# seveirbian/go-libp2p-pubsub

Measured on AMD Instinct MI355X. Metric: peer-message deliveries/sec + gossipsub rounds/sec (node), 1M peers 64 topics, higher is better.
Workload: dtype f64+u64; 1 GPU; config4: 1M peers, 64 topics, k=32, gossipsub v1.1 + Eth2 scoring, 1000 msgs/round, 10 hops/round; peers=1000000, topics=64, degree=32, msgs_per_round=1000, hops_per_round=10, parallelism=replicas1

## Files before the change

### go-libp2p-pubsub_amd/csrc/gs_engine.hip

```cpp
#include "gs_engine.h"

static thread_local std::string g_err;
void gs_set_error(const std::string& msg) { g_err = msg; }

static std::vector<int32_t> partition_bounds(const std::vector<int64_t>& rowptr, int N, int world) {
  const int64_t E = rowptr[N];
  std::vector<int32_t> part(world + 1, N);
  part[0] = 0;
  for (int r = 1; r < world; ++r)
    part[r] = (int32_t)(std::lower_bound(rowptr.begin(), rowptr.begin() + N, (E * r) / world) - rowptr.begin());
  for (int r = 1; r <= world; ++r) part[r] = std::max(part[r], part[r - 1]);
  return part;
}

static TopicP to_dev(const gs_topic_score_params& p, bool scored) {
  TopicP t{};
  t.TopicWeight = p.TopicWeight;
  t.TimeInMeshWeight = p.TimeInMeshWeight;
  t.TimeInMeshQuantum = p.TimeInMeshQuantum ? p.TimeInMeshQuantum : 1;
  t.TimeInMeshCap = p.TimeInMeshCap;
  t.FmdWeight = p.FirstMessageDeliveriesWeight;
  t.FmdDecay = p.FirstMessageDeliveriesDecay;
  t.FmdCap = p.FirstMessageDeliveriesCap;
  t.MmdWeight = p.MeshMessageDeliveriesWeight;
// ... 445 lines not shown
int gs_engine::allocIwantPool() {
  Dev& x = d;
  poolSeg = cfg.router == GS_ROUTER_GOSSIPSUB ? std::max<int64_t>((1 << 24) / world, 4 * eOwn) : 16;
  poolSeg = (poolSeg + 63) & ~63ll;
  x.poolCap = (int64_t)(rank + 1) * poolSeg;
  int sub = 1;
  while (world == 1 && sub < 256 && (poolSeg / (2 * sub)) >= (1 << 20)) sub *= 2;
  x.poolSub = sub;
  x.poolSubCap = poolSeg / sub;
  x.poolBase0 = (int64_t)rank * poolSeg;
  x.poolS0Mask = -1;
  if (const char* dbg = std::getenv("GS_DEBUG_POOL_SUB_CAP"))
    if (world == 1) {
      x.poolSubCap = std::min<int64_t>(x.poolSubCap, std::max<long long>(1, std::atoll(dbg)));
      x.poolS0Mask = 0;
      std::fprintf(stderr, "gossip engine: GS_DEBUG_POOL_SUB_CAP=%s active (IWANT sub-arenas of %lld ids, "
                   "sub-arena 0 first; a test-only setting)\n", dbg, (long long)x.poolSubCap);
    }
  for (int k = 0; k < 2; ++k) x.pool[k] = dalloc<int32_t>((size_t)poolSeg * world);
  x.poolCnt = dalloc<unsigned long long>((size_t)2 * x.poolSub * 16);
  x.cutSpK = dalloc<unsigned long long>(GS_CUTSPILL); x.cutSpM = dalloc<int64_t>(GS_CUTSPILL);
  x.cutSpN = dalloc<unsigned long long>(1);
  if (doPX) {
    for (int k = 0; k < 2; ++k) x.cPx[k] = ralloc<int64_t>(0xFF);
    x.pxqCap = std::max<int64_t>(1 << 16, 4 * (int64_t)N);
    x.pxq = dalloc<unsigned long long>((size_t)x.pxqCap); x.pxqN = dalloc<unsigned long long>(1);
  }
  x.slotSrc = dalloc<int32_t>(S, 0xFF); x.slotPubHop = dalloc<int64_t>(S); x.slotMid = dalloc<int64_t>(S, 0xFF);
  x.slotKind = dalloc<uint8_t>(S);
  return GS_OK;
}

int gs_engine::allocAdversary(const Plan& pl) {
  Dev& x = d;
  if (!behaveAll) return GS_OK;
  uint8_t* b = dalloc<uint8_t>(N);
  GS_TRY(putNow(b, behaveH.data(), (size_t)N));
  x.behave = b;
  if (!(behaveAll & GS_BEHAVE_IWANT_SPAM)) return GS_OK;
  for (int k = 0; k < 2; ++k) {
    x.cSpam[k] = ralloc<int64_t>(0xFF);
    x.cNSrv[k] = ralloc<uint8_t>();
  }
  x.pmaskRow = dalloc<int32_t>(N);
  x.pmask = dalloc<uint64_t>((size_t)pl.nSpam * S);
  x.spamRow = ealloc<int32_t>();
  for (int k = 0; k < 2; ++k) x.pflag[k] = dalloc<uint8_t>((size_t)poolSeg * world);
  x.spamCnt = dalloc<uint32_t>((size_t)std::max<int64_t>(pl.nSpamEdges, 1) * (S / 8));
  GS_TRY(putNow(x.pmaskRow, pl.pmaskRowH.data(), (size_t)N));
  return putEdges(x.spamRow, spamRowH);
}

int gs_engine::allocGater(const Plan& pl) {
  Dev& x = d;
  if (!gaterOn) return GS_OK;
  x.gThreshold = gaterP.Threshold; x.gGlobalDecay = gaterP.GlobalDecay; x.gSourceDecay = gaterP.SourceDecay;
  x.gDecayToZero = gaterP.DecayToZero; x.gDupW = gaterP.DuplicateWeight; x.gIgnW = gaterP.IgnoreWeight;
  x.gRejW = gaterP.RejectWeight; x.gQuiet = gaterP.Quiet;
  x.gValidate = dalloc<double>(N); x.gThrottle = dalloc<double>(N); x.gLast = dalloc<int64_t>(N);
  x.gSt = ealloc<double>(0, 4);
  x.gGrp = ealloc<uint8_t>();
  x.gConn = ealloc<int32_t>(); x.gExp = ealloc<int64_t>();
  std::vector<uint8_t> grp(E);
  for (int u = 0; u < N; ++u)
    for (int64_t e = rowptr[u]; e < rowptr[u + 1]; ++e) {
      const uint32_t ip = ipv4.empty() ? 0u : ipv4[col[e]];
      int64_t f = rowptr[u];
      while ((ipv4.empty() ? 0u : ipv4[col[f]]) != ip) ++f;
      grp[e] = (uint8_t)(f - rowptr[u]);
    }
  std::vector<int64_t> never(N, INT64_MIN);
  std::vector<int32_t> conn((size_t)E, 0);
  for (int u = 0; u < N; ++u)
    for (int64_t e = rowptr[u]; e < rowptr[u + 1]; ++e)
      if (!pl.isDown(e)) conn[rowptr[u] + grp[e]]++;
  GS_TRY(putEdges(x.gConn, conn));
  GS_TRY(putEdges(x.gGrp, grp));
  return putNow(x.gLast, never.data(), (size_t)N);
}

int gs_engine::allocReadback() {
  Dev& x = d;
#ifdef GS_STAMPS
  x.stamps = dalloc<unsigned long long>((size_t)(N / 1024 + 1) * 24);
#endif
  x.pad = dalloc<double>(256 * 64 * 2);
  x.ctr = dalloc<unsigned long long>((size_t)C_NCOUNTERS * GS_CTR_SPREAD); x.err = dalloc<int32_t>(1);
  dScoreTmp = ealloc<double>();
  dHopOut = dalloc<int32_t>(N); dFromOut = dalloc<int32_t>(N);
  return GS_OK;
}

int gs_engine::allocLatency() {
  if (!latOn) return GS_OK;
  const size_t bins = (size_t)latBins();
  d.latCnt = dalloc<uint32_t>((size_t)S);
  dLatM = dalloc<uint32_t>((size_t)S * bins);
  dLatH = dalloc<unsigned long long>((size_t)T * bins);
  int cus = 0;
  HIPCHECK(hipDeviceGetAttribute(&cus, hipDeviceAttributeMultiprocessorCount, cfg.device));
  const unsigned fit = (unsigned)(GS_LAT_CU_LDS / std::max<size_t>((size_t)S * 4, 1));
  latGrid = std::min<unsigned>(std::max(fit, 1u), GS_LAT_WGS_PER_CU) * (unsigned)std::max(cus, 1);
  return GS_OK;
}

int gs_engine::allocTrace() {
  Dev& x = d;
  if (traceMask.empty()) return GS_OK;
  uint8_t* tm = dalloc<uint8_t>(N);
  x.trace = dalloc<gs_trace_event>((size_t)traceCap);
  x.traceN = dalloc<unsigned long long>(1);
  x.traceCap = traceCap;
  GS_TRY(putNow(tm, traceMask.data(), (size_t)N));
  x.traced = tm;
  for (int u = n0; u < n1; ++u) {
    if (!traceMask[u]) continue;
    auto up = [&](int64_t e) { return !dormant.count({std::min(u, col[e]), std::max(u, col[e])}); };
    for (int64_t e = rowptr[u]; e < rowptr[u + 1]; ++e)
      if (up(e))
        tracePending.push_back(gs_trace_event{0, -1, GS_TRACE_ADD_PEER, u, col[e], -1, 0, mixed ? protoH[e] : (uint8_t)0});
    for (int t = 0; t < T; ++t)
      if ((sub[u] >> t) & 1) tracePending.push_back(gs_trace_event{0, -1, GS_TRACE_JOIN, u, -1, (int16_t)t, 0, 0});
    for (int64_t e = rowptr[u]; e < rowptr[u + 1]; ++e)
      if (up(e)) hostRpc(GS_TRACE_RECV_RPC, u, col[e], 0, GS_RPC_ORD(0, GS_RPC_O_HELLO), -1, sub[col[e]], 1);
  }
  return GS_OK;
}

int gs_engine::allocPartition() {
  Dev& x = d;
  if (world == 1) return GS_OK;
  x.xmark = ealloc<uint8_t>();
  uint8_t* nr = dalloc<uint8_t>(N);
  xCnt = dalloc<unsigned long long>(gsx::XCnt::words(world));
  xOff = dalloc<int64_t>(world);
  xpCnt = dalloc<unsigned long long>(gsx::XpCnt::words(world));
  xpOff = dalloc<int64_t>(gsx::XpOff::words(world));
  std::vector<uint8_t> h(N);
  for (int r = 0; r < world; ++r)
    for (int v = part[r]; v < part[r + 1]; ++v) h[v] = (uint8_t)r;
  GS_TRY(putNow(nr, h.data(), (size_t)N));
  x.nodeRank = nr;
  HIPCHECK(hipHostMalloc((void**)&xHost, gsx::Readback::words(world) * 8, hipHostMallocDefault));
  return GS_OK;
}

int gs_engine::initConnections(const Plan& pl) {
  if (!events.empty() || doPX || !dormant.empty()) GS_TRY(enableChurn());
  if (dormant.empty()) return GS_OK;
  std::vector<uint8_t> al((size_t)E, 1);
  for (int64_t e = 0; e < E; ++e)
    if (pl.downH[e]) al[e] = aliveH[e] = 0;
  GS_TRY(putNow(d.alive, al.data(), (size_t)E));
  if (d.rstate) GS_TRY(putNow(d.rstate, al.data(), (size_t)E));
  return GS_OK;
}

int gs_engine::allocAcct(const Plan& pl) {
  Dev& x = d;
  if (!acctOn) return GS_OK;
  x.rpcB = ealloc<unsigned long long>(); x.rpcN = ealloc<unsigned long long>();
  AcctT* ac = dalloc<AcctT>(T);
  GS_TRY(allocFail("RPC accounting"));
  const uint64_t bo = (uint64_t)(gp.PruneBackoff / kSec);
  std::vector<AcctT> ah(T);
  for (int t = 0; t < T; ++t) {
    ah[t].msgF = (int32_t)gs_pb_field(acctMsg[t]);
// ... 1610 lines not shown
```

### go-libp2p-pubsub_amd/csrc/gs_kernels.h

```cpp
#pragma once
#include <type_traits>

#include "gs_device.h"

#define GS_SB 8
#ifndef GS_RB
#define GS_RB 4
#endif
#define GS_RP 1024
__device__ __forceinline__ int rp_pad(int pl) { return pl + (pl >> 6); }
__host__ __device__ __forceinline__ int score_wave_edges(int T) { return T * 64 <= GS_RP ? 64 : GS_RP / T; }
#define GS_SCW 256
template <int MODE, bool LANE_T>
__global__ __launch_bounds__(64) void k_score_rows(Dev d, double* __restrict__ out) {
  __shared__ double sT[GS_RP + GS_RP / 64];
  __shared__ uint16_t sList[GS_SCW];
  const int lane = lane_id();
  const int T = d.T;
  const int sgw = score_wave_edges(T);
  const int64_t eb = d.e0 + (int64_t)blockIdx.x * GS_SCW;
  int nNeed = 0;
#pragma unroll
  for (int k = 0; k < GS_SCW / 64; ++k) {
    const int64_t e = eb + 64 * k + lane;
// ... 444 lines not shown
  const int slot = d.mSlot[b + i];
  atomicOr((unsigned long long*)&d.pubmask[cur][slot >> 6], 1ull << (slot & 63));
}

__device__ __forceinline__ void rs_select(const Dev& d, int u, int64_t base, int deg, int p, uint64_t subp, int slot,
                                          int ff) {
  const int lane = lane_id();
  const int t = slot / d.St;
  const int origin = d.slotSrc[slot];
  const bool cand = lane < deg && ((subp >> t) & 1) && lane != ff && p != origin;
  const bool fs = cand && d.proto != nullptr && d.proto[base + lane] == GS_PROTO_FLOODSUB;
  const bool rc = cand && !fs;
  const int n = __popcll(__ballot(rc));
  bool sel = cand;
  if (n > 6) {
    int target = d.rsTarget < n ? d.rsTarget : n;
    if (target < n) {
      const uint64_t key = gs_key64(d.seed, GS_SITE_RANDOMSUB, u, (uint32_t)d.slotMid[slot], p, 0);
      sel = fs || select_k(rc, key, target);
    }
  }
  const unsigned long long m = __ballot(sel);
  if (lane == 0) d.sel[(int64_t)u * d.S + slot] = m;
}
__device__ __forceinline__ void rs_select2(const Dev& d, int u, int64_t base, int deg, int pIn, uint64_t subpIn,
                                           int slotA, int ffA, int slotB, int ffB) {
  const int lane = lane_id();
  const int h = lane >> 5, el = lane & 31;
  const int p = __shfl(pIn, el);
  const uint64_t subp = shfl_u64(subpIn, el);
  const int slot = h ? slotB : slotA;
  const int ff = h ? ffB : ffA;
  const int t = slot / d.St;
  const int origin = d.slotSrc[slot];
  const bool cand = el < deg && ((subp >> t) & 1) && el != ff && p != origin;
  const bool fs = cand && d.proto != nullptr && d.proto[base + el] == GS_PROTO_FLOODSUB;
  const bool rc = cand && !fs;
  const int n = __popc((uint32_t)(__ballot(rc) >> (32 * h)));
  bool sel = cand;
  const int target = d.rsTarget < n ? d.rsTarget : n;
  if (n > 6 && target < n) {
    const uint64_t key = gs_key64(d.seed, GS_SITE_RANDOMSUB, u, (uint32_t)d.slotMid[slot], p, 0);
    sel = fs || select_k_half(rc, key, target);
  }
  const unsigned long long m = __ballot(sel);
  if (lane == 0) d.sel[(int64_t)u * d.S + slotA] = m & 0xFFFFFFFFull;
  if (lane == 32) d.sel[(int64_t)u * d.S + slotB] = m >> 32;
}

struct WMask {
  uint64_t m[4];
};
__device__ __forceinline__ bool wm_has(const WMask& a, int w) { return (a.m[w >> 6] >> (w & 63)) & 1; }
__device__ __forceinline__ int wm_rank(const WMask& a, int w) {
  int r = 0;
  for (int k = 0; k < (w >> 6); ++k) r += __popcll(a.m[k]);
  return r + __popcll(a.m[w >> 6] & ((1ull << (w & 63)) - 1));
}

__device__ __forceinline__ unsigned long long wave_sum_ll(long long v) {
  for (int o = 32; o > 0; o >>= 1) v += __shfl_xor(v, o);
  return (unsigned long long)v;
}

#define GS_NO_SLOT 0x7FFFFFFF

#ifdef GS_STAMPS
#define GS_STAMP_AT(region, k, val)                                                                \
  do {                                                                                             \
    if ((blockIdx.x & 1023) == 0 && lane == 0) {                                                   \
      const int64_t _i = ((int64_t)d.N / 1024 + 1) * 8 * (region) + (blockIdx.x >> 10) * 8 + (k);  \
      if ((k) >= 0 && (k) < 8 && _i < ((int64_t)d.N / 1024 + 1) * 24) d.stamps[_i] = (val);        \
      else set_err(d, E_STAMP);                                                                    \
    }                                                                                              \
  } while (0)
#define GS_STAMP(k) GS_STAMP_AT(0, k, clock64())
#define GS_STAMPB(k) GS_STAMP_AT(1, k, clock64())
#define GS_STAMPH(k, v) GS_STAMP_AT(2, k, v)
#define GS_STAMPB_CLEAR()                                  \
  do {                                                     \
    for (int _k = 0; _k < 8; ++_k) GS_STAMP_AT(1, _k, 0ull); \
  } while (0)
#define GS_CLK() clock64()
#else
#define GS_STAMPH(k, v) \
  do {                  \
  } while (0)
#define GS_CLK() 0ull
#define GS_STAMP(k) \
  do {              \
  } while (0)
#define GS_STAMPB(k) \
  do {               \
  } while (0)
#define GS_STAMPB_CLEAR() \
  do {                    \
  } while (0)
#endif

template <bool ADV>
using PhaseADev = std::conditional_t<ADV, const Dev*, Dev>;
__device__ __forceinline__ const Dev& dev_of(const Dev& d) { return d; }
__device__ __forceinline__ const Dev& dev_of(const Dev* d) { return *d; }
#ifndef GS_WPE_PA_WIDE
#define GS_WPE_PA_WIDE 4
#endif
template <bool NARROW, bool ADV>
constexpr int pa_waves = (!NARROW && !ADV) ? GS_WPE_PA_WIDE : GS_WPE_PA;
template <int WPL, bool NARROW, bool ADV, bool DENSE = false>
__global__ __launch_bounds__(64) __attribute__((amdgpu_waves_per_eu(pa_waves<NARROW, ADV>))) void k_phase_a(
    PhaseADev<ADV> dArg, int64_t h, int cur, int head,
                                                WMask amR, WMask amW, WMask amP, WMask amF, int nR, int nY) {
  static_assert(!(DENSE && ADV), "the dense pass 1 is honest-only");
  const Dev& d = dev_of(dArg);
  extern __shared__ __attribute__((aligned(16))) uint32_t smem32[];
  const int nCnt = (d.T * d.maxDeg + 7) & ~7;
  const int nCntW = NARROW ? nCnt / 2 : nCnt;
  uint32_t* scnt = smem32;
  uint64_t* sD = (uint64_t*)(scnt + nCntW);
  const int cT = d.T;
  auto cword = [&](int i, int t) -> int { return NARROW ? (i * cT + t) >> 1 : i * cT + t; };
  uint64_t* sYm = sD + nR;
  uint16_t* sRk = (uint16_t*)(sYm + nR);
  uint16_t* sYp = sRk + d.W;
  uint8_t* sFirst = (uint8_t*)(sYm + nR) + ((2 * (d.W + nR) + 15) & ~15);
  uint32_t* sUnc = (uint32_t*)(sFirst + nY);
  const int prow = (ADV && d.pmaskRow != nullptr) ? d.pmaskRow[d.n0 + blockIdx.x] : -1;
  const bool hasUnc = d.needAge || (ADV && d.pmaskRow != nullptr);
  uint32_t* sInv = sUnc + (hasUnc ? nCnt : 0);
  uint32_t* sPer = sInv + nCnt;
  double* sGThr = (double*)(sPer + 4 * 64);
  uint64_t* sDrop = (uint64_t*)(sGThr + 64);
  __shared__ uint64_t sStart[GS_BMAP];
  __shared__ uint64_t sComp[64];
  __shared__ uint64_t sRelay[64], sPub[64];
  __shared__ int sSnd[64];
  __shared__ uint32_t sAddr[64];
  __shared__ uint32_t sQ[GS_QCAP];
  const int v = d.n0 + blockIdx.x;
  const int lane = lane_id();
  const int prv = cur ^ 1;
  const int W = d.W;
  const int T = d.T;
  const int FC = d.FC;
  const int64_t base = d.rowptr[v];
  const int deg = (int)(d.rowptr[v + 1] - base);
  const uint64_t sv = d.sub[v];
  const bool valid = lane < deg;
  const bool gossipV = gossip_host(d, v);
  const bool scoring = d.scoring != 0 && gossipV;
  int u = 0, jr = -1, Ln = 0;
  int64_t pOff = -1;
  uint64_t relay = 0, pub = 0, relayAll = 0, pubAll = 0;
  bool gray = false;
  int irOff = 0, irN = 0;
  if (valid) {
    const int64_t e = base + lane;
    u = d.col[e];
    jr = d.jrIn[e];
    const ulonglong2 fw = d.fwdIn[prv][e];
    relayAll = fw.x;
    pubAll = fw.y;
    relay = relayAll & sv;
    pub = pubAll & sv;
    const int64_t ir = d.cIresp[prv][e];
    if (ir >= 0) {
      irOff = (int)(ir >> 24);
      irN = (int)(ir & 0xFFFFFF);
    }
    gray = scoring && !d.direct[e] && d.score0[e] < d.graylistThr;
    if (relayAll | pubAll) {
      if (d.ibxRec[0] != nullptr) {
        const int64_t rec = d.ibxRec[prv][e];
        if (rec >= 0) {
          pOff = rec >> 24;
          Ln = (int)(rec & 0xFFFFFF);
        }
      }
      if (pOff < 0) Ln = d.fln[prv][u];
    }
  }
  bool liveD = false, authU = false;
  int exD = 0;
  if constexpr (DENSE) {
    authU = valid && d.nAuth[u] > 0;
    if (valid && (relayAll | pubAll)) {
      liveD = d.fbN[prv][u] != 0 && (relayAll != 0 || authU);
      exD = d.fex[prv][d.rev[base + lane]];
    }
    Ln = 0;
  }
  const uint64_t authM = __ballot(authU);
  const uint64_t pushM = __ballot(pOff >= 0);
  GS_STAMP(0);
  const bool authV = d.nAuth[v] > 0;
  for (int k = lane; k < nCntW / 4; k += 64) ((uint4*)scnt)[k] = make_uint4(0, 0, 0, 0);
  const bool acct = d.rpcB != nullptr;
  if (hasUnc)
    for (int k = lane; k < nCnt / 4; k += 64) ((uint4*)sUnc)[k] = make_uint4(0, 0, 0, 0);
  for (int k = lane; k < nR; k += 64) {
    sD[k] = 0;
    sYm[k] = d.yTab[k];
    sYp[k] = (uint16_t)d.yTab[d.W + k];
  }
  {
    int rb = 0;
#pragma unroll
    for (int j = 0; j < GS_MAX_WPL; ++j) {
      const uint64_t m = amR.m[j];
      if (64 * j + lane < W)
        sRk[64 * j + lane] = ((m >> lane) & 1) ? (uint16_t)(rb + __popcll(m & ((1ull << lane) - 1))) : (uint16_t)0xFFFF;
      rb += __popcll(m);
    }
  }
  for (int k = lane; k < nY / 16; k += 64) ((uint4*)sFirst)[k] = make_uint4(~0u, ~0u, ~0u, ~0u);
  bool ctlGated = false;
  int nSrvRpc = 0;
  if constexpr (ADV) {
    for (int k = lane; k < nCnt / 4; k += 64) ((uint4*)sInv)[k] = make_uint4(0, 0, 0, 0);
    for (int k = lane; k < 4 * 64; k += 64) sPer[k] = 0;
    for (int k = lane; k < nR; k += 64) sDrop[k] = 0;
    double thr = -1.0;
    if (d.gater && gossipV && valid && !gray && !d.direct[base + lane]) {
      const int64_t last = d.gLast[v];
      const double gv = d.gValidate[v], gt = d.gThrottle[v];
      const bool active = !(last == INT64_MIN || h * d.hop_ns - last > d.gQuiet) && gt != 0 &&
                          !(gv != 0 && gt / gv < d.gThreshold);
      if (active) {
        const int64_t ge = base + d.gGrp[base + lane];
        const double de = d.gSt[ge], du = d.gSt[d.eOwn + ge], ig = d.gSt[2 * d.eOwn + ge], rj = d.gSt[3 * d.eOwn + ge];
        const double total = de + d.gDupW * du + d.gIgnW * ig + d.gRejW * rj;
        if (total != 0) thr = (1 + de) / (1 + total);
      }
    }
    sGThr[lane] = thr;
    if (valid && thr >= 0 && (d.cPre[prv][base + lane] != 0 || d.cHb[prv][base + lane] != 0)) {
      const double uu = gs_key_to_unit(gs_key64(d.seed, GS_SITE_GATER, v, u, (uint32_t)h, 0xFFFFFFFFu));
      ctlGated = !(uu < thr);
    }
    if (valid && d.cNSrv[prv] != nullptr) nSrvRpc = d.cNSrv[prv][base + lane];
    else if (irN) nSrvRpc = 1;
  }
  constexpr int EPBP = 8;
  const int nb = pOff >= 0 ? (Ln + EPBP - 1) / EPBP : (Ln + 3) >> 2;
  const int bincl = wave_incl_sum(nb);
  const int totalBlk = wave_last(bincl);
  const int nNE = __popcll(__ballot(nb > 0));
  {
    const uint64_t ne = __ballot(nb > 0);
    for (int k = lane; k < GS_BMAP; k += 64) sStart[k] = 0ull;
    __syncthreads();
    const int fb = bincl - nb;
    if (nb > 0) {
      sComp[__popcll(ne & ((1ull << lane) - 1))] =
          (uint64_t)(unsigned)fb | ((uint64_t)lane << 24) | ((uint64_t)(unsigned)Ln << 32);
      if (fb < 64 * GS_BMAP) atomicOr((unsigned long long*)&sStart[fb >> 6], 1ull << (fb & 63));
    }
  }
  sRelay[lane] = relay;
  sPub[lane] = pub;
  sSnd[lane] = valid ? (u | (jr << 24) | (rs_host(d, u) ? (1 << 30) : 0) | (gray ? (1 << 31) : 0)) : 0;
  sAddr[lane] = pOff >= 0 ? (uint32_t)(pOff >> 3) : (uint32_t)u * (uint32_t)FC;
  const uint64_t scoredT = __ballot(lane < T && scoring && d.tp[lane].scored);
  constexpr int PF3 = 16;
  const int nWdPf = (NARROW && scoring && d.dltN != nullptr) ? (deg * T) >> 1 : 0;
  const bool pf3 = nWdPf > 0 && nWdPf <= 64 * PF3;
  uint32_t q3[PF3];
  if (pf3) {
    const uint32_t* const pw = (const uint32_t*)(d.dltN + base * T);
#pragma unroll
    for (int k = 0; k < PF3; ++k) {
      const int wi = lane + 64 * k;
      q3[k] = pw[wi < nWdPf ? wi : nWdPf - 1];
    }
  }
  uint64_t Sp[WPL], Hp[WPL], Op[WPL];
#pragma unroll
  for (int j = 0; j < WPL; ++j) {
    const int w = lane + 64 * j;
    Sp[j] = Hp[j] = Op[j] = 0;
    if constexpr (!ADV) {
      const bool act = w < W && wm_has(amR, w);
      if (act || (w < W && wm_has(amP, w))) Sp[j] = d.seen[(int64_t)v * W + w];
      if (act) {
        Op[j] = d.oldm[w];
        if (gossipV) Hp[j] = d.hist[((int64_t)head * d.nOwnH + (v - d.n0)) * W + w];
      }
    }
  }
  __syncthreads();
  GS_STAMP(1);

  int nSent = 0, nGray = 0;
  long long nCopies = 0;
  int nGatedCopies = 0;
  uint64_t throttled = 0;
  auto kindOf = [&](int slot, int t) -> int {
    if constexpr (!ADV) return GS_MSG_VALID;
    return ((d.topicVal >> t) & 1) ? (int)d.slotKind[slot] : GS_MSG_VALID;
  };
  auto gated = [&](int i, int slot) -> bool {
    if constexpr (!ADV) return false;
    const double thr = sGThr[i];
    if (thr < 0) return false;
    const uint32_t mid = (uint32_t)d.slotMid[slot];
    const double uu = gs_key_to_unit(gs_key64(d.seed, GS_SITE_GATER, v, d.col[base + i], (uint32_t)h, mid));
    return !(uu < thr);
  };
  const bool trv = is_traced(d, v);
  auto deliver = [&](int i, int slot, bool payloadRpc) {
    if (payloadRpc && gated(i, slot)) {
      ++nGatedCopies;
      throttled |= 1ull << i;
      return;
    }
    const int w = slot >> 6;
    const int t = (int)__umulhi((unsigned)slot, d.stMagic);
    if (trv) trace_emit(d, h, GS_TRACE_COPY, v, d.col[base + i], t, d.slotMid[slot], 2);
    const int kind = kindOf(slot, t);
    if constexpr (ADV) {
      atomicAdd(&sPer[i], 1u);
      if (kind == GS_MSG_REJECT) atomicAdd(&sInv[i * T + t], 1u);
    }
    if (kind == GS_MSG_VALID) {
      if (NARROW) {
        const int pl = i * T + t;
        atomicAdd(&scnt[cword(i, t)], 1u << (16 * (pl & 1)));
      } else {
        atomicAdd(&scnt[cword(i, t)], 1u);
      }
    }
    ++nCopies;
    const int rk = sRk[w];
    const uint64_t ym = rk == 0xFFFF ? 0ull : sYm[rk];
    const bool young = (ym >> (slot & 63)) & 1;
    unsigned long long pold = 0;
    if (prow >= 0 && kind == GS_MSG_VALID)
      pold = atomicOr((unsigned long long*)&d.pmask[(int64_t)prow * d.S + slot], 1ull << i);
    if (d.needAge || !young || prow >= 0) {
      const bool had = (d.seen[(int64_t)v * W + w] >> (slot & 63)) & 1;
      if (had && kind == GS_MSG_VALID) {
        bool unc = (pold >> i) & 1;
        if (d.needAge && !unc) {
          const int64_t firstHop = d.slotPubHop[slot] + d.age[(int64_t)v * d.S + slot];
          unc = (h - firstHop) * d.hop_ns > d.tp[t].MmdWindow;
        }
        if (unc) atomicAdd(&sUnc[i * T + t], 1u);
      }
      if (!young) {
        if (!had) set_err(d, E_LATE);
        return;
      }
    }
    const int ix = sYp[rk] + __popcll(ym & ((1ull << (slot & 63)) - 1));
    atomicOr((unsigned long long*)&sD[rk], 1ull << (slot & 63));
    uint32_t* wp = (uint32_t*)(sFirst + (ix & ~3));
    const int sh = 8 * (ix & 3);
    uint32_t old = *wp;
    while ((int)((old >> sh) & 0xFF) > i) {
      const uint32_t nw = (old & ~(0xFFu << sh)) | ((uint32_t)i << sh);
      const uint32_t prev = atomicCAS(wp, old, nw);
      if (prev == old) break;
      old = prev;
    }
  };
  const uint32_t* const flPrv = prv ? d.fl[1] : d.fl[0];
  const uint16_t* const ibxPrv = prv ? d.ibx[1] : d.ibx[0];
  auto load_block = [&](int i, int kb) -> uint4 {
    if ((pushM >> i) & 1) return *(const uint4*)(ibxPrv + 8 * (size_t)sAddr[i] + 8 * kb);
    return *(const uint4*)(flPrv + (size_t)sAddr[i] + 4 * kb);
  };
  auto walk = [&](auto&& fn, bool count) {
    int qh = 0, qt = 0;
    int rankPrev = -1;
    constexpr int PB = 8;
    for (int b0 = 0; b0 < totalBlk; b0 += 64 * PB) {
      int si[PB], kb[PB];
      uint4 q[PB];
#pragma unroll
      for (int rr = 0; rr < PB; ++rr) {
        const int B = b0 + rr * 64;
        const int bidx = B + lane;
        si[rr] = -1;
        kb[rr] = 0;
        q[rr] = make_uint4(0, 0, 0, 0);
        if (B < 64 * GS_BMAP) {
          const uint64_t mb = sStart[B >> 6];
          const int rank = rankPrev + __popcll(mb & ((2ull << lane) - 1));
          rankPrev += __popcll(mb);
          if (bidx < totalBlk) {
            const uint64_t ce = sComp[rank];
            si[rr] = (int)((ce >> 24) & 63);
            const int k = bidx - (int)(ce & 0xFFFFFF);
            kb[rr] = k | (int)((ce >> 32) << 16);
            q[rr] = load_block(si[rr], k);
          }
        } else if (bidx < totalBlk) {
          int lo = 0, hi = nNE - 1;
          while (lo < hi) {
            const int mid = (lo + hi + 1) >> 1;
            if ((int)(sComp[mid] & 0xFFFFFF) <= bidx) lo = mid; else hi = mid - 1;
          }
          const uint64_t ce = sComp[lo];
          si[rr] = (int)((ce >> 24) & 63);
          const int k = bidx - (int)(ce & 0xFFFFFF);
          kb[rr] = k | (int)((ce >> 32) << 16);
          q[rr] = load_block(si[rr], k);
        }
      }
#pragma unroll
      for (int rr = 0; rr < PB; ++rr) {
        if (b0 + rr * 64 >= totalBlk) break;
        uint32_t en[EPBP];
        bool sn[EPBP];
        bool wide = false;
        {
          const int i = si[rr] < 0 ? 0 : si[rr];
          const int snd = sSnd[i];
          const int uu = snd & 0xFFFFFF;
          const int jri = (snd >> 24) & 0x3F;
          const bool rsS = (snd >> 30) & 1;
          const bool isGray = snd < 0;
          const uint64_t rl = sRelay[i], pb = sPub[i];
          const bool pushed = (pushM >> i) & 1;
          const int epb = pushed ? EPBP : 4;
          const int n = si[rr] < 0 ? 0 : min(epb, (kb[rr] >> 16) - epb * (kb[rr] & 0xFFFF));
          wide = n > 4;
#pragma unroll
          for (int c = 4; c < EPBP; ++c) {
            sn[c] = false;
            en[c] = 0;
          }
          if (pushed) {
#pragma unroll
            for (int c = 0; c < EPBP; ++c) {
              const uint32_t wd = c < 2 ? q[rr].x : c < 4 ? q[rr].y : c < 6 ? q[rr].z : q[rr].w;
              const int slot = (int)((c & 1) ? (wd >> 16) : (wd & 0xFFFFu));
              const int t = (int)__umulhi((unsigned)slot, d.stMagic);
              const bool sent = c < n && !(authV && d.slotSrc[slot] == v);
              if (count) {
                nSent += sent;
                if (sent && isGray) ++nGray;
              }
              sn[c] = sent && !isGray && ((sv >> t) & 1);
              en[c] = (uint32_t)slot | ((uint32_t)i << 16);
            }
          } else {
#pragma unroll
          for (int c = 0; c < 4; ++c) {
            const uint32_t ent = c == 0 ? q[rr].x : (c == 1 ? q[rr].y : (c == 2 ? q[rr].z : q[rr].w));
            const int slot = (int)(ent & 0xFFFF);
            const int tag = (int)(ent >> 16);
            const int t = (int)__umulhi((unsigned)slot, d.stMagic);
            bool sent = c < n && (tag == 255 ? ((pb >> t) & 1) : ((rl >> t) & 1));
            sent = sent && tag != jri;
            if (sent && rsS) sent = (d.sel[(int64_t)uu * d.S + slot] >> jri) & 1;
            if (sent && authV && d.slotSrc[slot] == v) sent = false;
            if (count) {
              nSent += sent;
              if (sent && isGray) ++nGray;
            }
            sn[c] = sent && !isGray;
            en[c] = (uint32_t)slot | ((uint32_t)i << 16);
          }
          }
        }
        const bool wideAny = __ballot(wide) != 0;
#pragma unroll
        for (int g = 0; g < EPBP / 4; ++g) {
          if (g > 0 && !wideAny) break;
#pragma unroll
          for (int c = 4 * g; c < 4 * g + 4; ++c) {
            const uint64_t m = __ballot(sn[c]);
            if (sn[c]) sQ[qt + lane_rank(m)] = en[c];
            qt += __popcll(m);
          }
          __syncthreads();
          if (qt >= 64) {
            while (qt - qh >= 64) {
              const uint32_t ent = sQ[qh + lane];
              fn((int)(ent >> 16), (int)(ent & 0xFFFF));
              qh += 64;
            }
            const uint32_t rest = lane < qt - qh ? sQ[qh + lane] : 0u;
            __syncthreads();
            if (lane < qt - qh) sQ[lane] = rest;
            qt -= qh;
            qh = 0;
            __syncthreads();
          }
        }
      }
    }
    if (lane < qt - qh) {
      const uint32_t ent = sQ[qh + lane];
      fn((int)(ent >> 16), (int)(ent & 0xFFFF));
    }
    __syncthreads();
  };
  long long nValidated = 0, nRejected = 0, nThrottledCopies = 0;
  bool dropPass = false;
  auto drop = [&](int i, int slot, bool payloadRpc) {
    const int rk = sRk[slot >> 6];
    if (rk == 0xFFFF || !((sDrop[rk] >> (slot & 63)) & 1)) return;
    if (payloadRpc && gated(i, slot)) return;
    const int t = (int)__umulhi((unsigned)slot, d.stMagic);
    const int kind = kindOf(slot, t);
    atomicSub(&sPer[i], 1u);
    if (kind == GS_MSG_REJECT) atomicSub(&sInv[i * T + t], 1u);
    if (kind == GS_MSG_VALID) {
      if (NARROW) {
        const int pl = i * T + t;
        atomicSub(&scnt[cword(i, t)], 1u << (16 * (pl & 1)));
      } else {
        atomicSub(&scnt[cword(i, t)], 1u);
      }
    }
    ++nThrottledCopies;
    --nCopies;
    if (trv)
      trace_emit(d, h, GS_TRACE_REJECT_MESSAGE, v, d.col[base + i], t, d.slotMid[slot], 2, GS_REJECT_QUEUE_FULL);
  };
  auto onCopy = [&](int i, int slot) {
    if (ADV && dropPass) drop(i, slot, true);
    else deliver(i, slot, true);
  };
  if constexpr (DENSE) {
    int* const sLv = (int*)sComp;
    int* const sCs = (int*)sPub;
    const uint64_t lmD = __ballot(liveD);
    const int nLv = __popcll(lmD);
    if (liveD) sLv[__popcll(lmD & ((1ull << lane) - 1))] = lane;
    sCs[lane] = 0;
    const bool svT = sv & 1;
    __syncthreads();
    const uint64_t* const fbPrv = d.fb[prv];
    uint64_t lateM = 0;
    for (int r0 = 0; r0 < nR; r0 += 64) {
      const int k = r0 + lane;
      const bool act = k < nR;
      const int w = act ? (int)(d.yTab[W + k] >> 32) : 0;
      const uint64_t Y = act ? sYm[k] : 0ull;
      const uint64_t Sv = act ? d.seen[(int64_t)v * W + w] : 0ull;
      const uint64_t O = (act && authV) ? d.own[(int64_t)v * W + w] : 0ull;
      const int yp = act ? (int)sYp[k] : 0;
      uint64_t D = 0;
      for (int k0 = 0; k0 < nLv; k0 += 8) {
        uint64_t F[8];
#pragma unroll
        for (int q = 0; q < 8; ++q) {
          const int i = k0 + q < nLv ? sLv[k0 + q] : -1;
          F[q] = (i >= 0 && act) ? fbPrv[(int64_t)(sSnd[i] & 0xFFFFFF) * W + w] : 0ull;
        }
#pragma unroll
        for (int q = 0; q < 8; ++q) {
          if (k0 + q >= nLv) break;
          const int i = sLv[k0 + q];
          const bool r = lane_get64(relayAll, i) & 1, p = lane_get64(pubAll, i) & 1;
          uint64_t A = 0;
          if (r != p) {
            const int uq = sSnd[i] & 0xFFFFFF;
            if (d.nAuth[uq] > 0 && act) A = d.own[(int64_t)uq * W + w];
          }
          const uint64_t f = F[q];
          const uint64_t sb = (r ? (p ? f : f & ~A) : (p ? f & A : 0ull)) & ~O;
          const int cs = wave_last(wave_incl_sum(__popcll(sb)));
          if (lane == 0) sCs[i] += cs;
          if (!svT || sSnd[i] < 0) continue;
          lateM |= sb & ~Y & ~Sv;
          const uint64_t y = sb & Y;
          for (uint64_t nb = y & ~D & ~Sv; nb; nb &= nb - 1)
            sFirst[yp + __popcll(Y & ((1ull << (__ffsll((long long)nb) - 1)) - 1))] = (uint8_t)i;
          D |= y;
        }
      }
      if (act) sD[k] = D;
    }
    if (lateM) set_err(d, E_LATE);
    __syncthreads();
    if (liveD) {
      const int c = sCs[lane] - ((relayAll & 1) ? exD : 0);
      nSent += c;
      if (gray) {
        nGray += c;
      } else if (svT) {
        nCopies += c;
        if (c) atomicAdd(&scnt[cword(lane, 0)], NARROW ? (uint32_t)c << (16 * (lane & 1)) : (uint32_t)c);
      }
    }
    if (trv && valid && !gray && (relay | pub)) {
      const uint32_t* L = d.fl[prv] + (int64_t)u * FC;
      const int nL = d.fln[prv][u];
      for (int k = 0; k < nL; ++k) {
        const uint32_t ent = L[k];
        const int slot = (int)(ent & 0xFFFF), tag = (int)(ent >> 16);
        const int t = (int)__umulhi((unsigned)slot, d.stMagic);
        bool sent = tag == 255 ? ((pub >> t) & 1) : ((relay >> t) & 1);
        sent = sent && tag != jr;
        if (sent && authV && d.slotSrc[slot] == v) sent = false;
        if (sent) trace_emit(d, h, GS_TRACE_COPY, v, u, t, d.slotMid[slot], 2);
      }
    }
    __syncthreads();
  } else {
  walk(onCopy, true);
  if (__ballot(((relayAll | pubAll) & ~sv) != 0)) {
    const uint64_t ru = relayAll & ~sv, pu = pubAll & ~sv;
    if ((ru | pu) && valid && pOff < 0) {
// ... 555 lines not shown
    if (U) {
      if ((U & Ow[j]) || !wm_has(amW, w)) set_err(d, E_LATE);
      if (gossipV && Ud) d.hist[((int64_t)head * d.nOwnH + (v - d.n0)) * W + w] = Hw[j] | Ud;
      nDeliv += k;
      auto put = [&](int b, int64_t ph) {
        const int slot = w * 64 + b;
        const int ff = sFirst[fidx(rkw[j], b)];
        if (trv)
          trace_emit(d, h, GS_TRACE_DELIVER_MESSAGE, v, d.col[base + ff], (int)__umulhi((unsigned)slot, d.stMagic),
                     d.slotMid[slot], 2);
        if (pmRow != nullptr)
          atomicAnd((unsigned long long*)&pmRow[slot], ~(1ull << ff));
        if (DENSE && (!((authM >> ff) & 1) || d.slotSrc[slot] != (sSnd[ff] & 0xFFFFFF)))
          atomicAdd((int*)sStart + ff, 1);
        if (!noFwd) {
          if (rank < FC) Lv[rank] = (uint32_t)slot | ((uint32_t)ff << 16);
          else set_err(d, E_FCAP);
        }
        ++rank;
        if constexpr (ADV)
          if (latRow != nullptr) atomicAdd(&latRow[slot], 1u);
        if (needAge) ageRow[slot] = (int16_t)(h - ph);
        if (record) ffRow[slot] = (uint8_t)ff;
      };
      uint64_t y = Ud;
      if (needAge) {
        while (y) {
          int bs[4];
          int64_t ph[4];
#pragma unroll
          for (int q = 0; q < 4; ++q) {
            bs[q] = y ? __ffsll((long long)y) - 1 : -1;
            y &= y ? y - 1 : 0ull;
          }
#pragma unroll
          for (int q = 0; q < 4; ++q) ph[q] = bs[q] >= 0 ? pubHop[w * 64 + bs[q]] : 0;
#pragma unroll
          for (int q = 0; q < 4; ++q)
            if (bs[q] >= 0) put(bs[q], ph[q]);
        }
      } else {
        while (y) {
          const int b = __ffsll((long long)y) - 1;
          y &= y - 1;
          put(b, 0);
        }
      }
    }
    if (rsV) {
      unsigned long long lanesWith = __ballot(Ud != 0);
      while (lanesWith) {
        const int src = __ffsll((long long)lanesWith) - 1;
        lanesWith &= lanesWith - 1;
        uint64_t y = lane_get64(Ud, src);
        const int wsrc = src + 64 * j;
        const int rks = lane_get(rkw[j], src);
        while (y) {
          const int b = __ffsll((long long)y) - 1;
          y &= y - 1;
          const int slot = wsrc * 64 + b, ff = sFirst[fidx(rks, b)];
          if (!pair2) {
            rs_select(d, v, base, deg, rsP, rsSub, slot, ff);
          } else if (pendSlot < 0) {
            pendSlot = slot;
            pendFf = ff;
          } else {
            rs_select2(d, v, base, deg, rsP, rsSub, pendSlot, pendFf, slot, ff);
            pendSlot = -1;
          }
        }
      }
    }
  }
  if (pendSlot >= 0) rs_select(d, v, base, deg, rsP, rsSub, pendSlot, pendFf);
  GS_STAMP(4);
  if (lane == 0) d.fln[cur][v] = behaves(d, v, GS_BEHAVE_NO_FORWARD) ? 0 : (running < FC ? running : FC);
  if constexpr (DENSE) {
    __syncthreads();
    if (valid) d.fex[cur][base + lane] = ((const int*)sStart)[lane];
    if (lane == 0) d.fbN[cur][v] = running;
  }
  const long long deliv = (long long)wave_sum_ll(nDeliv);
  const unsigned long long copies = wave_sum_ll(nCopies), s2 = wave_sum_ll(nSent), s3 = wave_sum_ll(nGray);
  if (lane == 0) {
    if (deliv) ctr_add(d, C_DELIVERIES, (unsigned long long)deliv);
    if (s2) ctr_add(d, C_TRANSMISSIONS, s2);
    if (s3) ctr_add(d, C_GRAYLISTED, s3);
  }
  if constexpr (ADV) {
    const unsigned long long rej = wave_sum_ll(nRejected), thc = wave_sum_ll(nThrottledCopies);
    const unsigned long long gc = wave_sum_ll(nGatedCopies);
    if (lane == 0) {
      const unsigned long long dups = copies - (unsigned long long)deliv - rej;
      if (dups) ctr_add(d, C_DUPLICATES, dups);
      if (rej) ctr_add(d, C_REJECTED, rej);
      if (thc) ctr_add(d, C_THROTTLED, thc);
      if (gc) ctr_add(d, C_GATED, gc);
    }
  } else {
    if (lane == 0 && copies - deliv) ctr_add(d, C_DUPLICATES, copies - deliv);
  }
}

template <int WPL>
__global__ __launch_bounds__(64) void k_flood_a(Dev d, int64_t h, int cur, WMask amR, WMask amW, WMask amP) {
  __shared__ int sNb[64];
  __shared__ uint64_t sSubN[64];
  __shared__ int sAuth[64];
  __shared__ int sEx[64];
  __shared__ int sLive[64];
  const int v = d.n0 + blockIdx.x;
  const int lane = lane_id();
  const int prv = cur ^ 1;
  const int W = d.W, Wt = d.Wt;
  const int64_t base = d.rowptr[v];
  const int deg = (int)(d.rowptr[v + 1] - base);
  const uint64_t sv = d.sub[v];
  const bool valid = lane < deg;
  int ex = 0;
  bool live = false;
  if (valid) {
    const int64_t e = base + lane;
    const int u = d.col[e];
    sNb[lane] = u;
    sSubN[lane] = d.subA[u];
    sAuth[lane] = d.nAuth[u] > 0;
    ex = d.fex[prv][d.rev[e]];
    live = d.fbN[prv][u] != 0;
  }
  sEx[lane] = 0;
  const uint64_t lm = __ballot(live);
  const int nLive = __popcll(lm);
  if (live) sLive[__popcll(lm & ((1ull << lane) - 1))] = lane;
  const int oldN = d.fbN[cur][v];
  bool anyRet = false;
#pragma unroll
  for (int j = 0; j < GS_MAX_WPL; ++j) anyRet |= amP.m[j] != 0;
  if (nLive == 0 && !anyRet) {
    if (oldN != 0) {
      for (int w = lane; w < W; w += 64) d.fb[cur][(int64_t)v * W + w] = 0ull;
      if (lane == 0) d.fbN[cur][v] = 0;
    }
    if (valid) d.fex[cur][base + lane] = 0;
    return;
  }
  uint64_t acc[WPL], S[WPL], R[WPL], O[WPL];
  bool act[WPL];
#pragma unroll
  for (int j = 0; j < WPL; ++j) {
    const int w = lane + 64 * j;
    act[j] = w < W && wm_has(amR, w) && ((sv >> (w / Wt)) & 1);
    const bool ret = w < W && wm_has(amP, w);
    S[j] = (act[j] || ret) ? d.seen[(int64_t)v * W + w] : 0ull;
    O[j] = act[j] ? d.own[(int64_t)v * W + w] : 0ull;
    R[j] = ret ? d.pubmask[cur][w] : 0ull;
    acc[j] = 0;
  }
  __syncthreads();
  const uint64_t* const fbPrv = d.fb[prv];
  int16_t* const ageRow = d.needAge ? d.age + (int64_t)v * d.S : nullptr;
  uint8_t* const ffRow = d.record ? d.ffrom + (int64_t)v * d.S : nullptr;
  long long sent = 0;
  for (int k0 = 0; k0 < nLive; k0 += 4) {
    uint64_t F[4][WPL], A[4][WPL];
#pragma unroll
    for (int q = 0; q < 4; ++q) {
// ... 376 lines not shown
```

Before: 5.114 billion deliveries/s.

## Pre-mask young window with seen bits and tally copies at enqueue time

In the non-adversarial, non-dense path, the seen/old/history window is now prefetched before the shared tables are built. The young mask is stored already ANDed with the receiver's seen bits, and the prefix offsets are recomputed by a wave scan, so per-copy delivery usually skips the global seen-word lookup. A fast 'tally' path counts copies and marks already-seen ones at enqueue time, tagging queue entries so the drain only performs the first-arrival mark. It adds a slow-window fallback, extra registers and a wave scan, plus optional stamp counters under GS_STAMPS.

```diff
diff --git a/go-libp2p-pubsub_amd/csrc/gs_engine.hip b/go-libp2p-pubsub_amd/csrc/gs_engine.hip
--- a/go-libp2p-pubsub_amd/csrc/gs_engine.hip
+++ b/go-libp2p-pubsub_amd/csrc/gs_engine.hip
@@ -551,7 +551,7 @@
 int gs_engine::allocReadback() {
   Dev& x = d;
 #ifdef GS_STAMPS
-  x.stamps = dalloc<unsigned long long>((size_t)(N / 1024 + 1) * 24);
+  x.stamps = dalloc<unsigned long long>((size_t)(N / 1024 + 1) * 24 + 4);
 #endif
   x.pad = dalloc<double>(256 * 64 * 2);
   x.ctr = dalloc<unsigned long long>((size_t)C_NCOUNTERS * GS_CTR_SPREAD); x.err = dalloc<int32_t>(1);
diff --git a/go-libp2p-pubsub_amd/csrc/gs_kernels.h b/go-libp2p-pubsub_amd/csrc/gs_kernels.h
--- a/go-libp2p-pubsub_amd/csrc/gs_kernels.h
+++ b/go-libp2p-pubsub_amd/csrc/gs_kernels.h
@@ -550,6 +550,11 @@
     for (int _k = 0; _k < 8; ++_k) GS_STAMP_AT(1, _k, 0ull); \
   } while (0)
 #define GS_CLK() clock64()
+#define GS_SEEN_COUNT(k, val)                                                                           \
+  do {                                                                                                  \
+    const unsigned long long _s = wave_sum_ll(val);                                                     \
+    if (lane == 0 && _s) atomicAdd(&d.stamps[((int64_t)d.N / 1024 + 1) * 24 + (k)], _s);                \
+  } while (0)
 #else
 #define GS_STAMPH(k, v) \
   do {                  \
@@ -662,15 +667,50 @@
   const uint64_t pushM = __ballot(pOff >= 0);
   GS_STAMP(0);
   const bool authV = d.nAuth[v] > 0;
+  constexpr bool UNSEEN = !ADV && !DENSE;
+  uint64_t Sp[WPL], Hp[WPL], Op[WPL];
+  auto prefetchWindow = [&]() {
+#pragma unroll
+    for (int j = 0; j < WPL; ++j) {
+      const int w = lane + 64 * j;
+      Sp[j] = Hp[j] = Op[j] = 0;
+      if constexpr (!ADV) {
+        const bool act = w < W && wm_has(amR, w);
+        if (act || (w < W && wm_has(amP, w))) Sp[j] = d.seen[(int64_t)v * W + w];
+        if (act) {
+          Op[j] = d.oldm[w];
+          if (gossipV) Hp[j] = d.hist[((int64_t)head * d.nOwnH + (v - d.n0)) * W + w];
+        }
+      }
+    }
+  };
+  if constexpr (UNSEEN) prefetchWindow();
   for (int k = lane; k < nCntW / 4; k += 64) ((uint4*)scnt)[k] = make_uint4(0, 0, 0, 0);
   const bool acct = d.rpcB != nullptr;
   if (hasUnc)
     for (int k = lane; k < nCnt / 4; k += 64) ((uint4*)sUnc)[k] = make_uint4(0, 0, 0, 0);
-  for (int k = lane; k < nR; k += 64) {
-    sD[k] = 0;
-    sYm[k] = d.yTab[k];
-    sYp[k] = (uint16_t)d.yTab[d.W + k];
-  }
+  bool slowL = false;
+  if constexpr (!UNSEEN) {
+    for (int k = lane; k < nR; k += 64) {
+      sD[k] = 0;
+      sYm[k] = d.yTab[k];
+      sYp[k] = (uint16_t)d.yTab[W + k];
+    }
+  } else {
+    for (int k = lane; k < nR; k += 64) sD[k] = 0;
+#pragma unroll
+    for (int j = 0; j < WPL; ++j) {
+      const int w = lane + 64 * j;
+      if (w < W && wm_has(amR, w)) {
+        const int rk = wm_rank(amR, w);
+        const uint64_t ym = d.yTab[rk];
+        sYm[rk] = ym & ~Sp[j];
+        const bool mine = (sv >> (int)__umulhi((unsigned)(w * 64), d.stMagic)) & 1;
+        slowL |= mine && (Op[j] & ~Sp[j] & ~ym) != 0;
+      }
+    }
+  }
+  const bool slowW = __ballot(slowL) != 0;
   {
     int rb = 0;
 #pragma unroll
@@ -742,18 +782,15 @@
       q3[k] = pw[wi < nWdPf ? wi : nWdPf - 1];
     }
   }
-  uint64_t Sp[WPL], Hp[WPL], Op[WPL];
-#pragma unroll
-  for (int j = 0; j < WPL; ++j) {
-    const int w = lane + 64 * j;
-    Sp[j] = Hp[j] = Op[j] = 0;
-    if constexpr (!ADV) {
-      const bool act = w < W && wm_has(amR, w);
-      if (act || (w < W && wm_has(amP, w))) Sp[j] = d.seen[(int64_t)v * W + w];
-      if (act) {
-        Op[j] = d.oldm[w];
-        if (gossipV) Hp[j] = d.hist[((int64_t)head * d.nOwnH + (v - d.n0)) * W + w];
-      }
+  if constexpr (!UNSEEN) prefetchWindow();
+  if constexpr (UNSEEN) {
+    int before = 0;
+    for (int r0 = 0; r0 < nR; r0 += 64) {
+      const int k = r0 + lane;
+      const int c = k < nR ? __popcll(sYm[k]) : 0;
+      const int incl = wave_incl_sum(c);
+      if (k < nR) sYp[k] = (uint16_t)(before + incl - c);
+      before += wave_last(incl);
     }
   }
   __syncthreads();
@@ -761,6 +798,9 @@
 
   int nSent = 0, nGray = 0;
   long long nCopies = 0;
+#ifdef GS_STAMPS
+  long long nSeenCopies = 0;
+#endif
   int nGatedCopies = 0;
   uint64_t throttled = 0;
   auto kindOf = [&](int slot, int t) -> int {
@@ -776,52 +816,17 @@
     return !(uu < thr);
   };
   const bool trv = is_traced(d, v);
-  auto deliver = [&](int i, int slot, bool payloadRpc) {
-    if (payloadRpc && gated(i, slot)) {
-      ++nGatedCopies;
-      throttled |= 1ull << i;
-      return;
-    }
-    const int w = slot >> 6;
-    const int t = (int)__umulhi((unsigned)slot, d.stMagic);
-    if (trv) trace_emit(d, h, GS_TRACE_COPY, v, d.col[base + i], t, d.slotMid[slot], 2);
-    const int kind = kindOf(slot, t);
-    if constexpr (ADV) {
-      atomicAdd(&sPer[i], 1u);
-      if (kind == GS_MSG_REJECT) atomicAdd(&sInv[i * T + t], 1u);
-    }
-    if (kind == GS_MSG_VALID) {
-      if (NARROW) {
-        const int pl = i * T + t;
-        atomicAdd(&scnt[cword(i, t)], 1u << (16 * (pl & 1)));
-      } else {
-        atomicAdd(&scnt[cword(i, t)], 1u);
-      }
-    }
-    ++nCopies;
-    const int rk = sRk[w];
-    const uint64_t ym = rk == 0xFFFF ? 0ull : sYm[rk];
-    const bool young = (ym >> (slot & 63)) & 1;
-    unsigned long long pold = 0;
-    if (prow >= 0 && kind == GS_MSG_VALID)
-      pold = atomicOr((unsigned long long*)&d.pmask[(int64_t)prow * d.S + slot], 1ull << i);
-    if (d.needAge || !young || prow >= 0) {
-      const bool had = (d.seen[(int64_t)v * W + w] >> (slot & 63)) & 1;
-      if (had && kind == GS_MSG_VALID) {
-        bool unc = (pold >> i) & 1;
-        if (d.needAge && !unc) {
-          const int64_t firstHop = d.slotPubHop[slot] + d.age[(int64_t)v * d.S + slot];
-          unc = (h - firstHop) * d.hop_ns > d.tp[t].MmdWindow;
-        }
-        if (unc) atomicAdd(&sUnc[i * T + t], 1u);
-      }
-      if (!young) {
-        if (!had) set_err(d, E_LATE);
-        return;
-      }
-    }
-    const int ix = sYp[rk] + __popcll(ym & ((1ull << (slot & 63)) - 1));
-    atomicOr((unsigned long long*)&sD[rk], 1ull << (slot & 63));
+  auto addCopy = [&](int i, int t) {
+    if (NARROW) {
+      const int pl = i * T + t;
+      atomicAdd(&scnt[cword(i, t)], 1u << (16 * (pl & 1)));
+    } else {
+      atomicAdd(&scnt[cword(i, t)], 1u);
+    }
+  };
+  auto mark = [&](int i, int rk, uint64_t ym, int b) {
+    const int ix = sYp[rk] + __popcll(ym & ((1ull << b) - 1));
+    atomicOr((unsigned long long*)&sD[rk], 1ull << b);
     uint32_t* wp = (uint32_t*)(sFirst + (ix & ~3));
     const int sh = 8 * (ix & 3);
     uint32_t old = *wp;
@@ -831,6 +836,65 @@
       if (prev == old) break;
       old = prev;
     }
+  };
+  auto deliver = [&](int i, int slot, bool payloadRpc) {
+    if (payloadRpc && gated(i, slot)) {
+      ++nGatedCopies;
+      throttled |= 1ull << i;
+      return;
+    }
+    const int w = slot >> 6;
+    const int t = (int)__umulhi((unsigned)slot, d.stMagic);
+    if (trv) trace_emit(d, h, GS_TRACE_COPY, v, d.col[base + i], t, d.slotMid[slot], 2);
+    const int kind = kindOf(slot, t);
+    if constexpr (ADV) {
+      atomicAdd(&sPer[i], 1u);
+      if (kind == GS_MSG_REJECT) atomicAdd(&sInv[i * T + t], 1u);
+    }
+    if (kind == GS_MSG_VALID) addCopy(i, t);
+    ++nCopies;
+    const int rk = sRk[w];
+    const uint64_t ym = rk == 0xFFFF ? 0ull : sYm[rk];
+    const bool open = (ym >> (slot & 63)) & 1;
+    unsigned long long pold = 0;
+    if (prow >= 0 && kind == GS_MSG_VALID)
+      pold = atomicOr((unsigned long long*)&d.pmask[(int64_t)prow * d.S + slot], 1ull << i);
+    if (UNSEEN ? !open : (d.needAge || !open || prow >= 0)) {
+      bool had = true;
+      if (!UNSEEN || slowW || rk == 0xFFFF) had = (d.seen[(int64_t)v * W + w] >> (slot & 63)) & 1;
+      if (had && kind == GS_MSG_VALID && (!UNSEEN || d.needAge || prow >= 0)) {
+        bool unc = (pold >> i) & 1;
+        if (d.needAge && !unc) {
+          const int64_t firstHop = d.slotPubHop[slot] + d.age[(int64_t)v * d.S + slot];
+          unc = (h - firstHop) * d.hop_ns > d.tp[t].MmdWindow;
+        }
+        if (unc) atomicAdd(&sUnc[i * T + t], 1u);
+      }
+#ifdef GS_STAMPS
+      nSeenCopies += had;
+#endif
+      if (!open) {
+        if (!had) set_err(d, E_LATE);
+        return;
+      }
+    }
+    mark(i, rk, ym, slot & 63);
+  };
+  constexpr uint32_t QCOUNTED = 1u << 31;
+  const bool tallyOn = !ADV && !trv && !d.needAge && !slowW;
+  auto tally = [&](int i, int slot, int t, uint32_t& ent) -> bool {
+    const int rk = sRk[slot >> 6];
+    if (rk == 0xFFFF) return true;
+    addCopy(i, t);
+    ++nCopies;
+    if (!((sYm[rk] >> (slot & 63)) & 1)) {
+#ifdef GS_STAMPS
+      ++nSeenCopies;
+#endif
+      return false;
+    }
+    ent |= QCOUNTED;
+    return true;
   };
   const uint32_t* const flPrv = prv ? d.fl[1] : d.fl[0];
   const uint16_t* const ibxPrv = prv ? d.ibx[1] : d.ibx[0];
@@ -912,6 +976,7 @@
               }
               sn[c] = sent && !isGray && ((sv >> t) & 1);
               en[c] = (uint32_t)slot | ((uint32_t)i << 16);
+              if (tallyOn && sn[c]) sn[c] = tally(i, slot, t, en[c]);
             }
           } else {
 #pragma unroll
@@ -947,7 +1012,7 @@
           if (qt >= 64) {
             while (qt - qh >= 64) {
               const uint32_t ent = sQ[qh + lane];
-              fn((int)(ent >> 16), (int)(ent & 0xFFFF));
+              fn((int)((ADV ? ent : ent & ~QCOUNTED) >> 16), (int)(ent & 0xFFFF), !ADV && (ent & QCOUNTED) != 0);
               qh += 64;
             }
             const uint32_t rest = lane < qt - qh ? sQ[qh + lane] : 0u;
@@ -962,7 +1027,7 @@
     }
     if (lane < qt - qh) {
       const uint32_t ent = sQ[qh + lane];
-      fn((int)(ent >> 16), (int)(ent & 0xFFFF));
+      fn((int)((ADV ? ent : ent & ~QCOUNTED) >> 16), (int)(ent & 0xFFFF), !ADV && (ent & QCOUNTED) != 0);
     }
     __syncthreads();
   };
@@ -989,9 +1054,15 @@
     if (trv)
       trace_emit(d, h, GS_TRACE_REJECT_MESSAGE, v, d.col[base + i], t, d.slotMid[slot], 2, GS_REJECT_QUEUE_FULL);
   };
-  auto onCopy = [&](int i, int slot) {
-    if (ADV && dropPass) drop(i, slot, true);
-    else deliver(i, slot, true);
+  auto onCopy = [&](int i, int slot, bool counted) {
+    if (ADV && dropPass) {
+      drop(i, slot, true);
+    } else if (counted) {
+      const int rk = sRk[slot >> 6];
+      mark(i, rk, sYm[rk], slot & 63);
+    } else {
+      deliver(i, slot, true);
+    }
   };
   if constexpr (DENSE) {
     int* const sLv = (int*)sComp;
@@ -1713,6 +1784,12 @@
   }
   const long long deliv = (long long)wave_sum_ll(nDeliv);
   const unsigned long long copies = wave_sum_ll(nCopies), s2 = wave_sum_ll(nSent), s3 = wave_sum_ll(nGray);
+#ifdef GS_STAMPS
+  GS_SEEN_COUNT(0, nCopies);
+  GS_SEEN_COUNT(1, nSeenCopies);
+  GS_SEEN_COUNT(2, lane == 0 ? 1ll : 0ll);
+  GS_SEEN_COUNT(3, lane == 0 && slowW ? 1ll : 0ll);
+#endif
   if (lane == 0) {
     if (deliv) ctr_add(d, C_DELIVERIES, (unsigned long long)deliv);
     if (s2) ctr_add(d, C_TRANSMISSIONS, s2);
```

New measurement: 5.108 billion deliveries/s. About the same (-0.1%).
